# boyuanf/tensorflow_train_distributed

Hardware: AMD Instinct MI355X
Metric: images/sec (whole node) ResNet-50 bf16 MirroredStrategy at 1/2/4/8 MI355X (higher is better)
Workload: dtype bf16; 1 GPU; model=ResNet-50 v1.5, global_batch=1024, per_gpu_batch=1024, image_size=224, parallelism=dp1, optimizer=momentum-SGD 0.9, wd 5e-5, fp32 master, precision=bf16, hipgraph=True

## Files before the change

tensorflow_train_distributed_amd/csrc/kernels/conv3_halo.hip:

```cpp
#include "stream_epi.h"

namespace ttdk {
namespace {
namespace c3 {

constexpr int THR = 512;
constexpr int NW = THR / 64;

struct Pro {
  const bf16_t* x;
  const bf16_t* x2;
  const uint8_t* mask;
  const float* s;
  const float* b;
  bf16_t* side;
  uint8_t* side_mask;
};

__device__ __forceinline__ void load8f(const float* p, float (&d)[8]) {
  const f32x4_t a = *reinterpret_cast<const f32x4_t*>(p), c = *reinterpret_cast<const f32x4_t*>(p + 4);
#pragma unroll
  for (int j = 0; j < 4; ++j) {
    d[j] = a[j];
    d[4 + j] = c[j];
  }
}

template <int CP>
__device__ __forceinline__ int slot_chunk(int q) { return (q >> 3) % CP; }
template <int CP>
__device__ __forceinline__ int slot_pix(int q) { return (q & 7) + 8 * (q / (8 * CP)); }

template <int C, int BN, int TH, int W, int PRO, bool FLIP, int WM>
__global__ __launch_bounds__(THR, 1) void conv3_kernel(Pro pa, const bf16_t* __restrict__ w, EpiParams E, int H,
                                                      int N, int tiles, int nslices) {
  constexpr int BM = TH * W;
  constexpr int HR = TH + 2, HC = W + 2;
  constexpr int CP = C / 8;
  constexpr int KT = 9 * C;
  constexpr int WN = NW / WM;
  constexpr int WR = BM / WM, WC = BN / WN;
  constexpr int TM = WR / 16, TN = WC / 16;
  constexpr int NPIX = HR * HC;
  constexpr int NCH = ((NPIX + 7) / 8) * 8 * CP;
  constexpr int NA = (NCH + THR - 1) / THR;
  constexpr int SB = BN * KT * 2;
  constexpr int REG = ((NPIX * 16 + 255) / 256) * 256;
  constexpr int SH = CP * REG;
  constexpr int PITCH = BN * 2 + 16;
  constexpr int SE = BM * PITCH + NW * 3 * BN * 4;
  constexpr int SAE = SH > SE ? SH : SE;
  static_assert(C % 64 == 0 && BN % 32 == 0 && WR % 16 == 0 && WC % 16 == 0, "tile shape");
  static_assert(THR % (8 * CP) == 0, "fixed channel chunk per thread");
  static_assert(SB + SAE <= 160 * 1024, "LDS budget");
  __shared__ __attribute__((aligned(16))) char smem[SB + SAE];
  char* const sB = smem;
  char* const sA = smem + SB;

  const int b = blockIdx.x;
  const int G = gridDim.x / nslices;
  const int xcd = b & 7, rq = b >> 3;
  const int slice = rq % nslices;
  const int per_xcd = G / 8;
  const int g = xcd * per_xcd + rq / nslices;
  const int n0 = slice * BN;
  const int tid = threadIdx.x, lane = tid & 63, wave = tid >> 6;
  const int wm = wave / WN, wn = wave % WN;
  const int tiles_per_img = H / TH;

  for (int q = tid; q < BN * (KT / 8); q += THR) {
    const int row = q / (KT / 8), kk = q % (KT / 8);
    const int tap = kk / CP, cc = kk % CP;
    const int n = n0 + row;
    const int src_tap = FLIP ? 8 - tap : tap;
    const uint4 v = n < N ? ldg16(w + (static_cast<long long>(n) * 9 + src_tap) * C + cc * 8) : make_uint4(0, 0, 0, 0);
    *reinterpret_cast<uint4*>(sB + (kk >> 3) * (BN * 128) + kmaj_off(row, kk & 7)) = v;
  }

  const int ac = slot_chunk<CP>(tid);
  const bool write_side = slice == 0 && pa.side != nullptr;

  const char* abase[TM];
#pragma unroll
  for (int a = 0; a < TM; ++a) {
    const int i = wm * WR + a * 16 + (lane & 15);
    abase[a] = sA + (lane >> 4) * REG + ((i / W) * HC + (i % W)) * 16;
  }

  uint4 ra[NA], rx[PRO == 2 ? NA : 1];
  uint32_t rm[(NA + 3) / 4];
  auto load_tile = [&](int t) {
    const int img = t / tiles_per_img, h0 = (t % tiles_per_img) * TH;
#pragma unroll
    for (int i = 0; i < (NA + 3) / 4; ++i) rm[i] = 0;
#pragma unroll
    for (int i = 0; i < NA; ++i) {
      const int pix = slot_pix<CP>(tid + THR * i);
      const int hr = pix / HC, hc = pix % HC;
      const int h = h0 - 1 + hr, x = hc - 1;
      const bool ok = pix < NPIX && h >= 0 && h < H && x >= 0 && x < W;
      const long long off = ((static_cast<long long>(img) * H + h) * W + x) * C + ac * 8;
      ra[i] = ok ? ldg16(pa.x + off) : make_uint4(0, 0, 0, 0);
      if constexpr (PRO == 2) {
        rx[i] = ok ? ldg16(pa.x2 + off) : make_uint4(0, 0, 0, 0);
        rm[i >> 2] |= static_cast<uint32_t>((ok && pa.mask) ? pa.mask[off >> 3] : 0xffu) << (8 * (i & 3));
      }
    }
  };
  auto stage_tile = [&](int t) {
    const int img = t / tiles_per_img, h0 = (t % tiles_per_img) * TH;
    float k0[8], k1[8], k2[8];
    if constexpr (PRO == 1) {
      load8f(pa.s + ac * 8, k0);
      load8f(pa.b + ac * 8, k1);
    } else if constexpr (PRO == 2) {
      load8f(pa.s + ac * 8, k0);
      load8f(pa.s + C + ac * 8, k1);
      load8f(pa.s + 2 * C + ac * 8, k2);
    }
#pragma unroll
    for (int i = 0; i < NA; ++i) {
      const int pix = slot_pix<CP>(tid + THR * i);
      if (tid + THR * i >= NCH) break;
      const int hr = pix / HC, hc = pix % HC;
      const int h = h0 - 1 + hr, x = hc - 1;
      const bool ok = h >= 0 && h < H && x >= 0 && x < W;
      const bool interior = ok && hr >= 1 && hr <= TH;
      const long long off = ((static_cast<long long>(img) * H + h) * W + x) * C + ac * 8;
      uint4 v = ra[i];
      if constexpr (PRO == 1) {
        float f[8];
        unpack8(ra[i], f);
#pragma unroll
        for (int j = 0; j < 8; ++j) f[j] = relu(f[j] * k0[j] + k1[j]);
        v = ok ? pack8(f) : make_uint4(0, 0, 0, 0);
        if (write_side && interior) {
          *reinterpret_cast<uint4*>(pa.side + off) = v;
          if (pa.side_mask) {
            const uint32_t wv[4] = {v.x, v.y, v.z, v.w};
            uint32_t mb = 0;
#pragma unroll
            for (int j = 0; j < 8; ++j) {
              const uint32_t hb = (wv[j >> 1] >> (16 * (j & 1))) & 0xffffu;
              mb |= ((hb & 0x7fffu) != 0 && !(hb & 0x8000u) ? 1u : 0u) << j;
            }
            pa.side_mask[off >> 3] = static_cast<uint8_t>(mb);
          }
        }
      } else if constexpr (PRO == 2) {
        float gq[8], yf[8];
        unpack8(ra[i], gq);
        const uint32_t mb = rm[i >> 2] >> (8 * (i & 3));
#pragma unroll
        for (int j = 0; j < 8; ++j) gq[j] = (mb >> j) & 1u ? gq[j] : 0.f;
        unpack8(rx[i], yf);
#pragma unroll
        for (int j = 0; j < 8; ++j) gq[j] = k0[j] * gq[j] + k1[j] * yf[j] + k2[j];
        v = ok ? pack8(gq) : make_uint4(0, 0, 0, 0);
        if (write_side && interior) *reinterpret_cast<uint4*>(pa.side + off) = v;
      }
      *reinterpret_cast<uint4*>(sA + ac * REG + pix * 16) = v;
    }
  };

  int t = g;
  if (t < tiles) load_tile(t);
  for (; t < tiles; t += G) {
    stage_tile(t);
    __syncthreads();
    if (t + G < tiles) load_tile(t + G);
    f32x4_t acc[TM][TN];
#pragma unroll
    for (int a = 0; a < TM; ++a)
#pragma unroll
      for (int c = 0; c < TN; ++c) acc[a][c] = f32x4_t{0.f, 0.f, 0.f, 0.f};
#pragma unroll
    for (int tap = 0; tap < 9; ++tap) {
      const int tq = (tap / 3) * HC + (tap % 3);
#pragma unroll
      for (int kc = 0; kc < C / 32; ++kc) {
        const int kglob = tap * C + kc * 32;
        const char* pB = sB + (kglob >> 6) * (BN * 128);
        const int kchunk = ((kglob & 63) >> 3) + (lane >> 4);
        bf16x8_t af[TM], bfr[TN];
#pragma unroll
        for (int c = 0; c < TN; ++c) bfr[c] = lds_read_b128(pB + kmaj_off(wn * WC + c * 16 + (lane & 15), kchunk));
#pragma unroll
        for (int a = 0; a < TM; ++a) af[a] = lds_read_b128(abase[a] + kc * 4 * REG + tq * 16);
#pragma unroll
        for (int a = 0; a < TM; ++a)
#pragma unroll
          for (int c = 0; c < TN; ++c) acc[a][c] = __builtin_amdgcn_mfma_f32_16x16x32_bf16(bfr[c], af[a], acc[a][c], 0, 0, 0);
      }
    }
    __syncthreads();
    sepi::stage_acc<TM, TN, WR, WC, PITCH>(sA, acc, wm, wn, lane, epi_alpha(E));
    __syncthreads();
    constexpr int ECPR = BN / 8;
    constexpr int RPP = THR / ECPR;
    const int m0 = t * BM;
    const int c = tid % ECPR, r0 = tid / ECPR;
    const int n = n0 + c * 8;
    const bool nfull = n + 8 <= N;
    const bool vst = nfull && (E.ldo & 7) == 0;
    float bias8[8], s8[8], q8[8], r8[8];
#pragma unroll
    for (int j = 0; j < 8; ++j) {
      bias8[j] = (E.bias && n + j < N) ? E.bias[n + j] : 0.f;
      s8[j] = q8[j] = r8[j] = 0.f;
    }
    const int M = tiles * BM;
    if (E.beta || E.residual || E.by)
      epi_rows<BM, RPP, PITCH, true, 2>(E, sA, c, r0, n, m0, M, N, vst, vst, bias8, s8, q8, r8);
    else
      epi_rows<BM, RPP, PITCH, false>(E, sA, c, r0, n, m0, M, N, vst, vst, bias8, s8, q8, r8);
    if (E.stat)
      sepi::tile_stats<BN, NW, THR, ECPR>(E, reinterpret_cast<float*>(sA + BM * PITCH), s8, q8, r8, c, lane, wave, tid,
                                          n0, N, t);
    else
      __syncthreads();
  }
}

template <int C, int BN, int TH, int W, int PRO, bool FLIP, int WM>
hipError_t launch(const Pro& pa, const bf16_t* w, const EpiParams& E, int Nimg, int H, int N, hipStream_t st) {
  const int nsl = N / BN;
  const int tiles = Nimg * (H / TH);
  int per_xcd = big::device_cus() / (8 * nsl);
  if (per_xcd < 1) per_xcd = 1;
  const int need = ceil_div(tiles, 8);
  if (per_xcd > need) per_xcd = need;
  hipLaunchKernelGGL((conv3_kernel<C, BN, TH, W, PRO, FLIP, WM>), dim3(8 * nsl * per_xcd), dim3(THR), 0, st, pa, w, E, H, N,
                     tiles, nsl);
  return hipGetLastError();
}

inline int pick_th(int C, int N, int W, int pro) {
  if (C == 64 && N == 64 && W == 56) return pro == 2 ? 4 : 8;
  return 0;
}

template <int PRO, bool FLIP>
hipError_t dispatch(const Pro& pa, const bf16_t* w, const EpiParams& E, int Nimg, int H, int W, int C, int N,
                    hipStream_t st) {
  if (C == 64 && N == 64 && W == 56) {
    if constexpr (PRO == 2) return launch<64, 64, 4, 56, PRO, FLIP, 2>(pa, w, E, Nimg, H, N, st);
    else return launch<64, 64, 8, 56, PRO, FLIP, 4>(pa, w, E, Nimg, H, N, st);
  }
  return hipErrorInvalidValue;
}

}

namespace c3s {

constexpr int THR = 512;
constexpr int NW = THR / 64;

__device__ __forceinline__ void dma16(const void* src, uint32_t lds_) {
  const uint32_t lds = __builtin_amdgcn_readfirstlane(lds_);
  unsigned keep;
  asm volatile("s_mov_b32 %0, m0\n\ts_mov_b32 m0, %2\n\ts_nop 0\n\tglobal_load_lds_dwordx4 %1, off\n\ts_mov_b32 m0, %0"
               : "=&s"(keep) : "v"(src), "s"(lds) : "memory");
}
__device__ __forceinline__ uint32_t lds_addr(const char* p) {
  typedef __attribute__((address_space(3))) const char lds_char_t;
  return (uint32_t)(size_t)(lds_char_t*)(p);
}

template <int N>
__device__ __forceinline__ void wait_vm() {
  asm volatile("s_waitcnt vmcnt(%0)" ::"n"(N) : "memory");
}

template <int C, int BN, int TR, int H, int W, int PRO, bool FLIP>
__global__ __launch_bounds__(THR, 1) void conv3s_kernel(c3::Pro pa, const bf16_t* __restrict__ w, EpiParams E,
                                                       int rows_total, int N, int tiles) {
  constexpr int WM = 2, WN = NW / WM;
  constexpr int BM = TR * W;
  constexpr int WR = BM / WM, WC = BN / WN;
  constexpr int TM = WR / 16, TN = WC / 16;
  constexpr int HS = TR + 4;
  constexpr int HC = W + 2;
  constexpr int NPIX = HS * HC;
  constexpr int CP = C / 8;
  constexpr int NCH = ((NPIX + 7) / 8) * 8 * CP;
  constexpr int NA = (NCH + THR - 1) / THR;
  constexpr int REG = ((NPIX * 16 + 255) / 256) * 256;
  constexpr int SH = CP * REG;
  constexpr int SBT = BN * C * 2;
  constexpr int PITCH = BN * 2 + 16;
  constexpr int SE = BM * PITCH + NW * 3 * BN * 4;
  constexpr int SAE = SH > SE ? SH : SE;
  constexpr int NDMA = SBT / 16 / THR;
  static_assert(PRO != 2 && C % 64 == 0 && BN % (16 * WN) == 0 && WR % 16 == 0 && TR <= H, "tile shape");
  static_assert(THR % (8 * CP) == 0 && SBT % (16 * THR) == 0, "staging / DMA mapping");
  static_assert(SAE + 2 * SBT <= 160 * 1024, "LDS budget");
  __shared__ __attribute__((aligned(16))) char smem[SAE + 2 * SBT];
  char* const sA = smem;
  char* const sBb = smem + SAE;

  const int b = blockIdx.x;
  const int G = gridDim.x;
  const int g = (b & 7) * (G / 8) + (b >> 3);
  const int tid = threadIdx.x, lane = tid & 63, wave = tid >> 6;
  const int wm = wave / WN, wn = wave % WN;
  const int ac = c3::slot_chunk<CP>(tid);
  const bool write_side = pa.side != nullptr;
  const int nimg = rows_total / H;

  auto dma_tap = [&](int tap, int buf) {
    const int stap = FLIP ? 8 - tap : tap;
    char* dst = sBb + buf * SBT;
#pragma unroll
    for (int i = 0; i < NDMA; ++i) {
      const int L = (i * NW + wave) * 64 + lane;
      const int sub = L / (BN * 8), p = L % (BN * 8), row = p >> 3, j = p & 7;
      const int sc = j ^ ((row >> 1) & 7);
      dma16(w + (static_cast<long long>(row) * 9 + stap) * C + (sub * 8 + sc) * 8,
            lds_addr(dst + (i * NW + wave) * 1024));
    }
  };
  struct Geo {
    int i0, h0, n0, n1;
  };
  auto geo = [&](int t) {
    Geo q;
    const int R0 = t * TR, R1 = min(R0 + TR, rows_total);
    q.i0 = R0 / H;
    q.h0 = R0 - q.i0 * H;
    q.n0 = min(R1, (q.i0 + 1) * H) - R0;
    q.n1 = R1 - R0 - q.n0;
    return q;
  };
  auto slot_src = [&](const Geo& q, int s, int& img, int& h, bool& interior) {
    if (s < q.n0 + 2) {
      img = q.i0;
      h = q.h0 - 1 + s;
      interior = s >= 1 && s <= q.n0;
      return true;
    }
    const int u = s - (q.n0 + 2);
    img = q.i0 + 1;
    h = u - 1;
    interior = u >= 1 && u <= q.n1;
    return q.n1 > 0 && u < q.n1 + 2;
  };

  uint4 ra[NA];
  auto load_tile = [&](int t) {
    const Geo q = geo(t);
#pragma unroll
    for (int i = 0; i < NA; ++i) {
      const int qq = tid + THR * i;
      const int pix = c3::slot_pix<CP>(qq);
      const int s = pix / HC, x = pix % HC - 1;
      int img, h;
      bool interior;
      const bool ok = qq < NCH && slot_src(q, s, img, h, interior) && h >= 0 && h < H && x >= 0 && x < W;
      const long long off = ((static_cast<long long>(img) * H + h) * W + x) * C + ac * 8;
      ra[i] = ldg16(ok ? pa.x + off : reinterpret_cast<const bf16_t*>(big::g_zero));
    }
  };
  auto stage_tile = [&](int t) {
    const Geo q = geo(t);
    float k0[8], k1[8];
    if constexpr (PRO == 1) {
      c3::load8f(pa.s + ac * 8, k0);
      c3::load8f(pa.b + ac * 8, k1);
    }
#pragma unroll
    for (int i = 0; i < NA; ++i) {
      const int qq = tid + THR * i;
      if (qq >= NCH) break;
      const int pix = c3::slot_pix<CP>(qq);
      const int s = pix / HC, x = pix % HC - 1;
      int img, h;
      bool interior;
      const bool ok = slot_src(q, s, img, h, interior) && h >= 0 && h < H && x >= 0 && x < W;
      uint4 v = ok ? ra[i] : make_uint4(0, 0, 0, 0);
      if constexpr (PRO == 1) {
        const long long off = ((static_cast<long long>(img) * H + h) * W + x) * C + ac * 8;
        float f[8];
        unpack8(ra[i], f);
#pragma unroll
        for (int j = 0; j < 8; ++j) f[j] = relu(f[j] * k0[j] + k1[j]);
        v = ok ? pack8(f) : make_uint4(0, 0, 0, 0);
        if (write_side && ok && interior) {
          *reinterpret_cast<uint4*>(pa.side + off) = v;
          if (pa.side_mask) {
            const uint32_t wv[4] = {v.x, v.y, v.z, v.w};
            uint32_t mb = 0;
#pragma unroll
            for (int j = 0; j < 8; ++j) {
              const uint32_t hb = (wv[j >> 1] >> (16 * (j & 1))) & 0xffffu;
              mb |= ((hb & 0x7fffu) != 0 && !(hb & 0x8000u) ? 1u : 0u) << j;
            }
            pa.side_mask[off >> 3] = static_cast<uint8_t>(mb);
          }
        }
      }
      *reinterpret_cast<uint4*>(sA + ac * REG + pix * 16) = v;
    }
  };

  int bcur = 0;
  int t = g;
  if (t < tiles) {
    dma_tap(0, 0);
    load_tile(t);
  }
  for (; t < tiles; t += G) {
    const Geo q = geo(t);
    int abase[TM];
#pragma unroll
    for (int a = 0; a < TM; ++a) {
      const int i = wm * WR + a * 16 + (lane & 15);
      const int j = i / W, col = i % W;
      abase[a] = (lane >> 4) * REG + ((j + (j >= q.n0 ? 2 : 0)) * HC + col) * 16;
    }
    stage_tile(t);
    wait_vm<0>();
    __syncthreads();
    const bool more = t + G < tiles;
    f32x4_t acc[TM][TN];
#pragma unroll
    for (int a = 0; a < TM; ++a)
#pragma unroll
      for (int c = 0; c < TN; ++c) acc[a][c] = f32x4_t{0.f, 0.f, 0.f, 0.f};
#pragma unroll 1
    for (int tap = 0; tap < 9; ++tap) {
      const int bnext = bcur ^ 1;
      if (tap < 8) dma_tap(tap + 1, bnext);
      else if (more) dma_tap(0, bnext);
      const char* sBc = sBb + bcur * SBT;
      const int tq = ((tap / 3) * HC + (tap % 3)) * 16;
#pragma unroll
      for (int kc = 0; kc < C / 32; ++kc) {
        const int kglob = kc * 32;
        const char* pB = sBc + (kglob >> 6) * (BN * 128);
        const int kchunk = ((kglob & 63) >> 3) + (lane >> 4);
        bf16x8_t af[TM], bfr[TN];
#pragma unroll
        for (int c = 0; c < TN; ++c) bfr[c] = lds_read_b128(pB + kmaj_off(wn * WC + c * 16 + (lane & 15), kchunk));
#pragma unroll
        for (int a = 0; a < TM; ++a) af[a] = lds_read_b128(sA + abase[a] + kc * 4 * REG + tq);
#pragma unroll
        for (int a = 0; a < TM; ++a)
#pragma unroll
          for (int c = 0; c < TN; ++c) acc[a][c] = __builtin_amdgcn_mfma_f32_16x16x32_bf16(bfr[c], af[a], acc[a][c], 0, 0, 0);
      }
      wait_vm<0>();
      __syncthreads();
      bcur = bnext;
    }
    sepi::stage_acc<TM, TN, WR, WC, PITCH>(sA, acc, wm, wn, lane, epi_alpha(E));
    if (more) load_tile(t + G);
    __syncthreads();
    constexpr int ECPR = BN / 8;
    constexpr int RPP = THR / ECPR;
    const int m0 = t * BM;
    const int c = tid % ECPR, r0 = tid / ECPR;
    const int n = c * 8;
    const bool vst = (E.ldo & 7) == 0;
    float bias8[8], s8[8], q8[8], r8[8];
#pragma unroll
    for (int j = 0; j < 8; ++j) {
      bias8[j] = E.bias ? E.bias[n + j] : 0.f;
      s8[j] = q8[j] = r8[j] = 0.f;
    }
    const int M = rows_total * W;
    if (E.beta || E.residual || E.by)
      epi_rows<BM, RPP, PITCH, true, 2>(E, sA, c, r0, n, m0, M, N, vst, vst, bias8, s8, q8, r8);
    else
      epi_rows<BM, RPP, PITCH, false>(E, sA, c, r0, n, m0, M, N, vst, vst, bias8, s8, q8, r8);
    if (E.stat)
      sepi::tile_stats<BN, NW, THR, ECPR>(E, reinterpret_cast<float*>(sA + BM * PITCH), s8, q8, r8, c, lane, wave, tid,
                                          0, N, t);
    else
      __syncthreads();
    (void)nimg;
  }
}

template <int PRO, bool FLIP>
hipError_t launch(const c3::Pro& pa, const bf16_t* w, const EpiParams& E, int Nimg, int N, hipStream_t st) {
  const int rows = Nimg * 28;
  const int tiles = ceil_div(rows, 8);
  int G = big::device_cus() / 8 * 8;
  if (G < 8) G = 8;
  const int need = ceil_div(tiles, 8) * 8;
  if (G > need) G = need;
  hipLaunchKernelGGL((conv3s_kernel<128, 128, 8, 28, 28, PRO, FLIP>), dim3(G), dim3(THR), 0, st, pa, w, E, rows, N,
                     tiles);
  return hipGetLastError();
}

inline bool fits(int H, int W, int C, int N, int pro) { return C == 128 && N == 128 && H == 28 && W == 28 && pro != 2; }

}
}
}

using namespace ttdk;

namespace {
int& conv3_s3_flag() {
  static int on = getenv_int("TTD_CONV3_S3", 1);
  return on;
}
}

TTDK_EXPORT int ttdk_set_conv3_s3(int on) {
  const int old = conv3_s3_flag();
  conv3_s3_flag() = on;
  return old;
}

TTDK_EXPORT int ttdk_conv3_rows(int H, int W, int C, int N, int pro) {
  if (conv3_s3_flag() && c3s::fits(H, W, C, N, pro)) return 8 * W;
  const int th = c3::pick_th(C, N, W, pro);
  return (th && H % th == 0) ? th * W : 0;
}

TTDK_EXPORT int ttdk_conv3_halo(const bf16_t* x, const bf16_t* x2, const uint8_t* mask_in, const float* s,
                                const float* b, bf16_t* side, uint8_t* side_mask, int pro, int flip, const bf16_t* w,
                                int Nimg, int H, int W, int C, int N, const TtdkEpilogue* epi, hipStream_t st) {
  if (ttdk_conv3_rows(H, W, C, N, pro) == 8 * W && c3s::fits(H, W, C, N, pro)) {
    if ((reinterpret_cast<uintptr_t>(x) & 15) || (reinterpret_cast<uintptr_t>(w) & 15)) return hipErrorInvalidValue;
    const EpiParams e = to_epi(epi);
    if (e.mode != 0 || e.remap || e.bH || e.ldo != N || e.residual || e.by2) return hipErrorInvalidValue;
    if (pro == 1 && (!s || !b)) return hipErrorInvalidValue;
    if (side_mask && pro != 1) return hipErrorInvalidValue;
    const c3::Pro pa{x, nullptr, nullptr, s, b, side, side_mask};
    if (pro == 0 && !flip) return c3s::launch<0, false>(pa, w, e, Nimg, N, st);
    if (pro == 0 && flip) return c3s::launch<0, true>(pa, w, e, Nimg, N, st);
    if (pro == 1 && !flip) return c3s::launch<1, false>(pa, w, e, Nimg, N, st);
    return hipErrorInvalidValue;
  }
  const int th = c3::pick_th(C, N, W, pro);
  if (!th || H % th || (reinterpret_cast<uintptr_t>(x) & 15) || pro < 0 || pro > 2) return hipErrorInvalidValue;
  const EpiParams e = to_epi(epi);
  if (e.mode != 0 || e.remap || e.bH || e.ldo != N || e.residual || e.by2) return hipErrorInvalidValue;
  if (pro == 1 && (!s || !b)) return hipErrorInvalidValue;
  if (pro == 2 && (!s || !x2)) return hipErrorInvalidValue;
  if (side_mask && pro != 1) return hipErrorInvalidValue;
  const c3::Pro pa{x, x2, mask_in, s, b, side, side_mask};
#define C3_CASE(P_, F_) \
  if (pro == P_ && (flip != 0) == F_) return c3::dispatch<P_, F_>(pa, w, e, Nimg, H, W, C, N, st);
  C3_CASE(0, false)
  C3_CASE(1, false)
  C3_CASE(0, true)
  C3_CASE(2, true)
#undef C3_CASE
  return hipErrorInvalidValue;
}
```

tensorflow_train_distributed_amd/ops/gemm.py:

```python
from __future__ import annotations

import ctypes

import torch

from . import _lib, _plan

ACT_NONE, ACT_RELU, ACT_GELU, ACT_TANH, ACT_DGELU = 0, 1, 2, 3, 4

import os as _os
_LOG = [] if _os.environ.get("TTD_GEMM_LOG") else None


def gemm_log(reset=False):
    out = list(_LOG or [])
    if reset and _LOG is not None:
        _LOG.clear()
    return out


def _log(kind, M, N, K, splits=1):
    if _LOG is not None:
        _LOG.append((kind, int(M), int(N), int(K), int(splits)))
    _lib.label((kind, int(M), int(N), int(K)))
# ... 67 lines not shown
        raise ValueError("gemm out must be [%d, %d] row-major (got %s strides %s)" % (M, N, tuple(out.shape),
                                                                                   out.stride()))
    _log("gemm_%s%s" % ("t" if trans_a else "n", "t" if trans_b else "n"), M, N, K, splits)
    a_kmajor = 0 if trans_a else 1
    lda = a.stride(0)
    b_kmajor = 1 if trans_b else 0
    ldb = b.stride(0)
    if out.dtype == torch.float32:
        splits = effective_splits(K, splits)
        if splits > 1:
            if not out.is_contiguous():
                raise ValueError("split-K output must be contiguous")
            ws = torch.empty((splits, M, N), dtype=torch.float32, device=a.device)
            _lib.call("ttdk_gemm_bf16_splitk", a.data_ptr(), lda, a_kmajor, b.data_ptr(), ldb, b_kmajor, M, N, K,
                      splits, ws.data_ptr(), out.data_ptr(), beta, float(alpha), int(tile[0]), int(tile[1]),
                      _lib.stream())
            return out
        e = _epi(out, mode=2, beta=beta, alpha=alpha)
    else:
        e = _epi(out, bias=bias, residual=residual, act=act, beta=beta, alpha=alpha, aux=aux, stat=stat)
    _lib.call("ttdk_gemm_bf16", a.data_ptr(), lda, a_kmajor, b.data_ptr(), ldb, b_kmajor, M, N, K, 1,
              tile[0], tile[1], ctypes.byref(e), _lib.stream())
    return out


_lib.register({"ttdk_gemm4w_bf16": [_lib.P, _lib.L, _lib.P, _lib.L, _lib.I, _lib.I, _lib.I, _lib.E, _lib.P],
               "ttdk_set_g4_sched": [_lib.I], "ttdk_set_g4_group": [_lib.I],
               "ttdk_set_g4_stagger": [_lib.I]})


def set_g4_stagger(v: int) -> int:
    return int(_lib.query("ttdk_set_g4_stagger", int(v)))


def set_g4_group(v: int) -> int:
    return int(_lib.query("ttdk_set_g4_group", int(v)))


def set_g4_sched(v: int) -> int:
    return int(_lib.query("ttdk_set_g4_sched", int(v)))


def gemm4w(a, b, *, out=None, bias=None, act=ACT_NONE, residual=None, beta=0, alpha=1.0, aux=None):
    _check2d(a, torch.bfloat16, "a")
    _check2d(b, torch.bfloat16, "b")
    M, K = a.shape
    N, Kb = b.shape
    if K != Kb:
        raise ValueError("gemm4w inner dims differ: %d vs %d" % (K, Kb))
    if out is None:
        out = torch.empty((M, N), dtype=torch.bfloat16, device=a.device)
    e = _epi(out, bias=bias, residual=residual, act=act, beta=beta, alpha=alpha, aux=aux)
    _log("gemm4w", M, N, K, 1)
    _lib.call("ttdk_gemm4w_bf16", a.data_ptr(), a.stride(0), b.data_ptr(), b.stride(0), M, N, K, ctypes.byref(e),
              _lib.stream())
    return out


_lib.register({"ttdk_gemm_bf16_batched": [_lib.P, _lib.L, _lib.L, _lib.I, _lib.P, _lib.L, _lib.L, _lib.I, _lib.P,
                                          _lib.L, _lib.L, _lib.I, _lib.I, _lib.I, _lib.I, _lib.I, _lib.P],
               "ttdk_gemm_f32_batched": [_lib.P, _lib.L, _lib.L, _lib.I, _lib.P, _lib.L, _lib.L, _lib.I, _lib.P,
                                         _lib.L, _lib.L, _lib.I, _lib.I, _lib.I, _lib.I, _lib.P]})


def gemm_batched(a, b, *, trans_a=False, trans_b=False, out_dtype=torch.float32):
    if a.dim() != 3 or b.dim() != 3 or a.shape[0] != b.shape[0]:
        raise ValueError("gemm_batched needs [B, ., .] operands with equal batch, got %s and %s"
                         % (tuple(a.shape), tuple(b.shape)))
    a = a.contiguous()
    b = b.contiguous()
    Bt = a.shape[0]
    M, K = (a.shape[2], a.shape[1]) if trans_a else (a.shape[1], a.shape[2])
    Kb, N = (b.shape[2], b.shape[1]) if trans_b else (b.shape[1], b.shape[2])
    if K != Kb:
        raise ValueError("gemm_batched inner dims differ: %d vs %d" % (K, Kb))
    _log("gemm_batched", M, N, K, Bt)
    if a.dtype == torch.float32 and b.dtype == torch.float32:
        out = torch.empty((Bt, M, N), dtype=torch.float32, device=a.device)
        _lib.call("ttdk_gemm_f32_batched", a.data_ptr(), a.stride(1), a.stride(0), int(trans_a), b.data_ptr(),
                  b.stride(1), b.stride(0), int(trans_b), out.data_ptr(), N, M * N, M, N, K, Bt, _lib.stream())
        return out
    _check(a, torch.bfloat16, "a")
    _check(b, torch.bfloat16, "b")
    out = torch.empty((Bt, M, N), dtype=out_dtype, device=a.device)
    _lib.call("ttdk_gemm_bf16_batched", a.data_ptr(), a.stride(1), a.stride(0), 0 if trans_a else 1, b.data_ptr(),
              b.stride(1), b.stride(0), 1 if trans_b else 0, out.data_ptr(), N, M * N,
              1 if out_dtype == torch.float32 else 0, M, N, K, Bt, _lib.stream())
    return out


def wgrad_bias_ok(M, N, K, splits) -> bool:
    if M % 8 or N % 8 or K % 64:
        return False
    if int(_lib.query("ttdk_gemm_wgrad_bias_ws", int(M), int(N), int(K), int(splits))) < 0:
        return False
    kt = K // 64
    return -(-kt // _plan.clamp_splits(kt, int(splits))) >= 16


def gemm_wgrad_bias(dy, x, out, bias_out, splits=1, beta=0, alpha=1.0):
    _check2d(dy, torch.bfloat16, "dy")
    _check2d(x, torch.bfloat16, "x")
    K, M = dy.shape
    K2, N = x.shape
    if K != K2:
        raise ValueError("gemm_wgrad_bias: token dims differ (%d vs %d)" % (K, K2))
    if tuple(out.shape) != (M, N) or out.dtype != torch.float32 or not out.is_contiguous():
        raise ValueError("gemm_wgrad_bias: out must be a contiguous fp32 [%d, %d]" % (M, N))
    if bias_out.numel() != M or bias_out.dtype != torch.float32 or not bias_out.is_contiguous():
        raise ValueError("gemm_wgrad_bias: bias_out must be a contiguous fp32 [%d]" % M)
    nws = int(_lib.query("ttdk_gemm_wgrad_bias_ws", M, N, K, int(splits)))
    if nws < 0:
        raise ValueError("gemm_wgrad_bias: shape %dx%dx%d not on the 256-wide kernel" % (M, N, K))
    ws = torch.empty(nws, dtype=torch.float32, device=dy.device)
    _log("wgrad_bias", M, N, K, splits)
    _lib.call("ttdk_gemm_wgrad_bias", dy.data_ptr(), dy.stride(0), x.data_ptr(), x.stride(0), M, N, K, int(splits),
              ws.data_ptr(), out.data_ptr(), int(beta), float(alpha), bias_out.data_ptr(), _lib.stream())
    return out, bias_out


def gemm4t(dy, x, out=None, bias_out=None, *, splits=1, beta=0, alpha=1.0):
    _check2d(dy, torch.bfloat16, "dy")
    _check2d(x, torch.bfloat16, "x")
    K, M = dy.shape
    K2, N = x.shape
    if K != K2:
        raise ValueError("gemm4t: token dims differ (%d vs %d)" % (K, K2))
    if out is None:
        out = torch.empty((M, N), dtype=torch.float32, device=dy.device)
    if tuple(out.shape) != (M, N) or out.dtype != torch.float32 or not out.is_contiguous():
        raise ValueError("gemm4t: out must be a contiguous fp32 [%d, %d]" % (M, N))
    if bias_out is not None and (bias_out.numel() != M or bias_out.dtype != torch.float32
                                 or not bias_out.is_contiguous()):
        raise ValueError("gemm4t: bias_out must be a contiguous fp32 [%d]" % M)
    nws = int(_lib.query("ttdk_gemm4t_ws", M, N, K, int(splits)))
    if nws < 0:
        raise ValueError("gemm4t does not take M=%d N=%d K=%d (K a multiple of 64 >= 128, M / N multiples "
                         "of 8, operands < 2 GiB, TTD_G4T on)" % (M, N, K))
    ws = torch.empty(max(nws, 1), dtype=torch.float32, device=dy.device)
    _log("gemm4t", M, N, K, splits)
    _lib.call("ttdk_gemm4t_wgrad", dy.data_ptr(), dy.stride(0), x.data_ptr(), x.stride(0), M, N, K, int(splits),
              ws.data_ptr(), out.data_ptr(), int(beta), float(alpha), _lib.ptr(bias_out), _lib.stream())
    return out


_C3 = _os.environ.get("TTD_CONV3", "1") != "0"


_lib.register({"ttdk_set_conv3_s3": [_lib.I]})


def set_conv3_s3(on: bool) -> bool:
    return bool(_lib.query("ttdk_set_conv3_s3", 1 if on else 0))


def conv3_rows(H, W, C, N, pro=0):
    return int(_lib.query("ttdk_conv3_rows", int(H), int(W), int(C), int(N), int(pro))) if _C3 else 0


def conv3_halo(x, w, *, prologue=None, flip=False, out=None, stat=False, bn_stat=None):
    _check(x, torch.bfloat16, "x")
    _check(w, torch.bfloat16, "w")
    Nimg, H, W, C = x.shape
    Co = w.shape[0]
    if tuple(w.shape) != (Co, 3, 3, C):
        raise ValueError("conv3_halo: filter must be [%d, 3, 3, %d], got %s" % (Co, C, tuple(w.shape)))
    pro_code = 0 if prologue is None else {"bn_fwd": 1, "bn_bwd": 2}.get(prologue[0], -1)
    bm = conv3_rows(H, W, C, Co, max(pro_code, 0))
    if not bm:
        raise ValueError("conv3_halo: shape %s -> %d not compiled in" % (tuple(x.shape), Co))
    if out is None:
        out = torch.empty((Nimg, H, W, Co), dtype=torch.bfloat16, device=x.device)
    T = -(-Nimg * H * W // bm)
    partial = None
    by = bmask = None
    if stat or bn_stat is not None:
        partial = torch.empty((T, 2, Co), dtype=torch.float32, device=x.device)
    if bn_stat is not None:
        by, bmask = bn_stat
        _check(by, torch.bfloat16, "bn_stat y")
    e = _epi(out, ldo=Co, stat=partial, by=by, bmask=bmask)
    P = _lib.ptr
    pro, x2, mask_in, s, b, side, side_mask = 0, None, None, None, None, None, None
    if prologue is not None:
        if prologue[0] == "bn_fwd":
            _, s, b, side, side_mask = prologue
            pro = 1
        elif prologue[0] == "bn_bwd":
            _, x2, mask_in, s, side = prologue
            pro = 2
        else:
            raise ValueError("unknown prologue %r" % (prologue[0],))
    _log("c3_%s" % ("dgrad" if flip else "fwd"), Nimg * H * W, Co, 9 * C)
    _lib.call("ttdk_conv3_halo", x.data_ptr(), P(x2), P(mask_in), P(s), P(b), P(side), P(side_mask), pro, int(flip),
              w.data_ptr(), Nimg, H, W, C, Co, ctypes.byref(e), _lib.stream())
    if partial is not None:
        return out, partial, T
    return out


def gemm_f32(a, b, *, trans_a=False, trans_b=False, out=None, bias=None, beta=0):
    _check2d(a, torch.float32, "a")
    _check2d(b, torch.float32, "b")
    M, K = (a.shape[1], a.shape[0]) if trans_a else a.shape
    Kb, N = (b.shape[1], b.shape[0]) if trans_b else b.shape
    if K != Kb:
        raise ValueError("gemm inner dims differ: %d vs %d" % (K, Kb))
    if out is None:
        if beta:
            raise ValueError("beta=1 needs an out tensor")
        out = torch.empty((M, N), dtype=torch.float32, device=a.device)
    elif out.dtype != torch.float32 or tuple(out.shape) != (M, N) or out.stride(-1) != 1:
        raise ValueError("gemm_f32 out must be fp32 [%d, %d] row-major" % (M, N))
    if bias is not None:
        _check(bias, torch.float32, "bias")
    _log("gemm_f32_%s%s" % ("t" if trans_a else "n", "t" if trans_b else "n"), M, N, K, 1)
    _lib.call("ttdk_gemm_f32", a.data_ptr(), a.stride(0), int(trans_a), b.data_ptr(), b.stride(0), int(trans_b),
              out.data_ptr(), out.stride(0), _lib.ptr(bias), int(bool(beta)), M, N, K, _lib.stream())
    return out


BIG_WGRAD_WGS = int(_os.environ.get("TTD_WGRAD_WGS", "128"))


def gemm_wgrad_splits(M, N, K, target_blocks=1024, min_ktiles=8, big_wgs=None):
    bbn = big_bn(M, N, K)
    if bbn:
        tiles = -(-M // 256) * -(-N // bbn)
        return max(1, min((K // 64) // 32, -(-(big_wgs or BIG_WGRAD_WGS) // tiles)))
    bm, bn = _plan.pick_tile(M, N)
    tiles = -(-M // bm) * -(-N // bn)
    ktiles = -(-K // 64)
    return max(1, min(ktiles // min_ktiles, -(-target_blocks // tiles)))


def conv_geom(x_shape, w_shape, stride, padding, dilation=(1, 1)):
    N, H, W, C = x_shape
    K, R, S, Cw = w_shape
    if C != Cw:
        raise ValueError("channel mismatch %d vs %d" % (C, Cw))
    sh, sw = stride
    ph, pw = padding
    dh, dw = dilation
    P = (H + 2 * ph - dh * (R - 1) - 1) // sh + 1
    Q = (W + 2 * pw - dw * (S - 1) - 1) // sw + 1
    g = _lib.ConvGeom(N, H, W, C, K, R, S, P, Q, sh, sw, ph, pw, dh, dw)
    return g


def pw_rows(N, K, dma=False):
    return int(_lib.query("ttdk_pw_rows", int(N), int(K), int(bool(dma))))


_PW = _os.environ.get("TTD_PW", "1") != "0"


def pw_ok(M, N, K):
    return _PW and pw_rows(N, K) > 0 and N * K <= 65536


def pw_wgrad_fusable(M, N, K, dma=True):
    return _PW and int(_lib.query("ttdk_pw_wgrad_slabs", int(M), int(N), int(K), int(bool(dma)), 0)) > 0


def pw_conv(x, w, *, prologue=None, out=None, stat=False, beta=0, residual=None, bn_stat=None, bn_stat2=None,
            beta_s2=None, wgrad=None, max_wgs=0, fold_stream=None, keep=None):
    _check(x, torch.bfloat16, "x")
    _check(w, torch.bfloat16, "w")
    K = x.shape[-1]
    M = x.numel() // K
    N = w.shape[0]
    if w.numel() != N * K:
        raise ValueError("pw_conv: weight must be [N, K] = [%d, %d] (got %s)" % (N, K, tuple(w.shape)))
    dma = bool(beta or bn_stat is not None) and residual is None and bn_stat2 is None
    bm = pw_rows(N, K, dma)
    if not bm:
        raise ValueError("pw_conv: N=%d K=%d not handled by the streaming kernel" % (N, K))
    if out is None:
        out = torch.empty(tuple(x.shape[:-1]) + (N,), dtype=torch.bfloat16, device=x.device)
    T = -(-M // bm)
    partial = partial2 = None
    by = bmask = by2 = None
    if stat or bn_stat is not None:
        partial = torch.empty((T, 2, N), dtype=torch.float32, device=x.device)
    if bn_stat is not None:
        by, bmask = bn_stat
        _check(by, torch.bfloat16, "bn_stat y")
        if bn_stat2 is not None:
            by2 = bn_stat2
            partial2 = torch.empty((T, 2, N), dtype=torch.float32, device=x.device)
    e = _epi(out, ldo=N, beta=beta, residual=residual, stat=partial, by=by, bmask=bmask, by2=by2, stat2=partial2,
             beta_s2=beta_s2 if beta else None)
    P = _lib.ptr
    pro, x2, mask_in, s, b, rs, rb, side, side_mask = 0, None, None, None, None, None, None, None, None
    if prologue is not None:
        if prologue[0] == "bn_fwd":
            _, s, b, x2, rs, rb, side, side_mask = prologue
            pro = 1
        elif prologue[0] == "bn_bwd":
            _, x2, mask_in, s, side = prologue
            pro = 2
        else:
            raise ValueError("pw_conv: unknown prologue %r" % (prologue[0],))
    _log("pw_%s" % ("fwd" if pro != 2 else "dgrad"), M, N, K)
    if wgrad is not None:
        xw, dw = wgrad[0], wgrad[1]
# ... 571 lines not shown
```

Baseline: 15620 images/sec.

## Interleave next-tile halo loads across conv3 taps and pin fragment scheduling

Adds a SCHED template variant (on by default via TTD_CONV3_SCHED) to the 3x3 halo conv kernels. In the stride kernel it spreads the next tile's halo global loads across the nine tap iterations, issuing two slots per tap, with partial vmcnt waits in place of a bulk load after the MMA loop. It also precomputes per-lane weight DMA source pointers. Both kernels insert sched_barrier fences around LDS fragment reads and MFMA groups, and use an opaque tid to stop the compiler hoisting address math. The aim is to hide global load latency behind the tap loop and keep register pressure steady. The risks are extra register use from full unrolling and weaker compiler scheduling.

```diff
diff --git a/tensorflow_train_distributed_amd/csrc/kernels/conv3_halo.hip b/tensorflow_train_distributed_amd/csrc/kernels/conv3_halo.hip
--- a/tensorflow_train_distributed_amd/csrc/kernels/conv3_halo.hip
+++ b/tensorflow_train_distributed_amd/csrc/kernels/conv3_halo.hip
@@ -31,7 +31,21 @@
 template <int CP>
 __device__ __forceinline__ int slot_pix(int q) { return (q & 7) + 8 * (q / (8 * CP)); }
 
-template <int C, int BN, int TH, int W, int PRO, bool FLIP, int WM>
+template <int SCHED>
+__device__ __forceinline__ int fresh(int tid) {
+  if constexpr (SCHED != 0) {
+    asm volatile("" : "+v"(tid));
+    __builtin_assume(tid >= 0 && tid < THR);
+  }
+  return tid;
+}
+
+template <int SCHED>
+__device__ __forceinline__ void frag_fence() {
+  if constexpr (SCHED != 0) __builtin_amdgcn_sched_barrier(0);
+}
+
+template <int C, int BN, int TH, int W, int PRO, bool FLIP, int WM, int SCHED>
 __global__ __launch_bounds__(THR, 1) void conv3_kernel(Pro pa, const bf16_t* __restrict__ w, EpiParams E, int H,
                                                       int N, int tiles, int nslices) {
   constexpr int BM = TH * W;
@@ -91,11 +105,12 @@
   uint32_t rm[(NA + 3) / 4];
   auto load_tile = [&](int t) {
     const int img = t / tiles_per_img, h0 = (t % tiles_per_img) * TH;
+    const int ft = fresh<SCHED>(tid);
 #pragma unroll
     for (int i = 0; i < (NA + 3) / 4; ++i) rm[i] = 0;
 #pragma unroll
     for (int i = 0; i < NA; ++i) {
-      const int pix = slot_pix<CP>(tid + THR * i);
+      const int pix = slot_pix<CP>(ft + THR * i);
       const int hr = pix / HC, hc = pix % HC;
       const int h = h0 - 1 + hr, x = hc - 1;
       const bool ok = pix < NPIX && h >= 0 && h < H && x >= 0 && x < W;
@@ -118,10 +133,11 @@
       load8f(pa.s + C + ac * 8, k1);
       load8f(pa.s + 2 * C + ac * 8, k2);
     }
+    const int ft = fresh<SCHED>(tid);
 #pragma unroll
     for (int i = 0; i < NA; ++i) {
-      const int pix = slot_pix<CP>(tid + THR * i);
-      if (tid + THR * i >= NCH) break;
+      const int pix = slot_pix<CP>(ft + THR * i);
+      if (ft + THR * i >= NCH) break;
       const int hr = pix / HC, hc = pix % HC;
       const int h = h0 - 1 + hr, x = hc - 1;
       const bool ok = h >= 0 && h < H && x >= 0 && x < W;
@@ -184,13 +200,20 @@
         const int kchunk = ((kglob & 63) >> 3) + (lane >> 4);
         bf16x8_t af[TM], bfr[TN];
 #pragma unroll
-        for (int c = 0; c < TN; ++c) bfr[c] = lds_read_b128(pB + kmaj_off(wn * WC + c * 16 + (lane & 15), kchunk));
-#pragma unroll
-        for (int a = 0; a < TM; ++a) af[a] = lds_read_b128(abase[a] + kc * 4 * REG + tq * 16);
+        for (int c = 0; c < TN; ++c) {
+          bfr[c] = lds_read_b128(pB + kmaj_off(wn * WC + c * 16 + (lane & 15), kchunk));
+          frag_fence<SCHED>();
+        }
+#pragma unroll
+        for (int a = 0; a < TM; ++a) {
+          af[a] = lds_read_b128(abase[a] + kc * 4 * REG + tq * 16);
+          frag_fence<SCHED>();
+        }
 #pragma unroll
         for (int a = 0; a < TM; ++a)
 #pragma unroll
           for (int c = 0; c < TN; ++c) acc[a][c] = __builtin_amdgcn_mfma_f32_16x16x32_bf16(bfr[c], af[a], acc[a][c], 0, 0, 0);
+        frag_fence<SCHED>();
       }
     }
     __syncthreads();
@@ -222,7 +245,7 @@
   }
 }
 
-template <int C, int BN, int TH, int W, int PRO, bool FLIP, int WM>
+template <int C, int BN, int TH, int W, int PRO, bool FLIP, int WM, int SCHED>
 hipError_t launch(const Pro& pa, const bf16_t* w, const EpiParams& E, int Nimg, int H, int N, hipStream_t st) {
   const int nsl = N / BN;
   const int tiles = Nimg * (H / TH);
@@ -230,8 +253,8 @@
   if (per_xcd < 1) per_xcd = 1;
   const int need = ceil_div(tiles, 8);
   if (per_xcd > need) per_xcd = need;
-  hipLaunchKernelGGL((conv3_kernel<C, BN, TH, W, PRO, FLIP, WM>), dim3(8 * nsl * per_xcd), dim3(THR), 0, st, pa, w, E, H, N,
-                     tiles, nsl);
+  hipLaunchKernelGGL((conv3_kernel<C, BN, TH, W, PRO, FLIP, WM, SCHED>), dim3(8 * nsl * per_xcd), dim3(THR), 0, st, pa, w,
+                     E, H, N, tiles, nsl);
   return hipGetLastError();
 }
 
@@ -240,12 +263,12 @@
   return 0;
 }
 
-template <int PRO, bool FLIP>
+template <int PRO, bool FLIP, int SCHED>
 hipError_t dispatch(const Pro& pa, const bf16_t* w, const EpiParams& E, int Nimg, int H, int W, int C, int N,
                     hipStream_t st) {
   if (C == 64 && N == 64 && W == 56) {
-    if constexpr (PRO == 2) return launch<64, 64, 4, 56, PRO, FLIP, 2>(pa, w, E, Nimg, H, N, st);
-    else return launch<64, 64, 8, 56, PRO, FLIP, 4>(pa, w, E, Nimg, H, N, st);
+    if constexpr (PRO == 2) return launch<64, 64, 4, 56, PRO, FLIP, 2, SCHED>(pa, w, E, Nimg, H, N, st);
+    else return launch<64, 64, 8, 56, PRO, FLIP, 4, SCHED>(pa, w, E, Nimg, H, N, st);
   }
   return hipErrorInvalidValue;
 }
@@ -272,8 +295,16 @@
 __device__ __forceinline__ void wait_vm() {
   asm volatile("s_waitcnt vmcnt(%0)" ::"n"(N) : "memory");
 }
-
-template <int C, int BN, int TR, int H, int W, int PRO, bool FLIP>
+__device__ __forceinline__ void wait_vm_upto(int n) {
+  switch (n) {
+    case 1: wait_vm<1>(); break;
+    case 2: wait_vm<2>(); break;
+    case 3: wait_vm<3>(); break;
+    default: wait_vm<0>(); break;
+  }
+}
+
+template <int C, int BN, int TR, int H, int W, int PRO, bool FLIP, int SCHED>
 __global__ __launch_bounds__(THR, 1) void conv3s_kernel(c3::Pro pa, const bf16_t* __restrict__ w, EpiParams E,
                                                        int rows_total, int N, int tiles) {
   constexpr int WM = 2, WN = NW / WM;
@@ -309,16 +340,30 @@
   const bool write_side = pa.side != nullptr;
   const int nimg = rows_total / H;
 
+  const bf16_t* wsrc[NDMA];
+#pragma unroll
+  for (int i = 0; i < NDMA; ++i) {
+    const int L = (i * NW + wave) * 64 + lane;
+    const int sub = L / (BN * 8), p = L % (BN * 8), row = p >> 3, j = p & 7;
+    const int sc = j ^ ((row >> 1) & 7);
+    wsrc[i] = w + static_cast<long long>(row) * 9 * C + (sub * 8 + sc) * 8;
+  }
   auto dma_tap = [&](int tap, int buf) {
     const int stap = FLIP ? 8 - tap : tap;
     char* dst = sBb + buf * SBT;
 #pragma unroll
     for (int i = 0; i < NDMA; ++i) {
-      const int L = (i * NW + wave) * 64 + lane;
-      const int sub = L / (BN * 8), p = L % (BN * 8), row = p >> 3, j = p & 7;
-      const int sc = j ^ ((row >> 1) & 7);
-      dma16(w + (static_cast<long long>(row) * 9 + stap) * C + (sub * 8 + sc) * 8,
-            lds_addr(dst + (i * NW + wave) * 1024));
+      if constexpr (SCHED != 0) {
+        int off = stap * C;
+        asm volatile("" : "+s"(off));
+        dma16(wsrc[i] + off, lds_addr(dst + (i * NW + wave) * 1024));
+      } else {
+        const int L = (i * NW + wave) * 64 + lane;
+        const int sub = L / (BN * 8), p = L % (BN * 8), row = p >> 3, j = p & 7;
+        const int sc = j ^ ((row >> 1) & 7);
+        dma16(w + (static_cast<long long>(row) * 9 + stap) * C + (sub * 8 + sc) * 8,
+              lds_addr(dst + (i * NW + wave) * 1024));
+      }
     }
   };
   struct Geo {
@@ -348,19 +393,21 @@
   };
 
   uint4 ra[NA];
+  auto load_slot = [&](const Geo& q, int ft, int i) {
+    const int qq = ft + THR * i;
+    const int pix = c3::slot_pix<CP>(qq);
+    const int s = pix / HC, x = pix % HC - 1;
+    int img, h;
+    bool interior;
+    const bool ok = qq < NCH && slot_src(q, s, img, h, interior) && h >= 0 && h < H && x >= 0 && x < W;
+    const long long off = ((static_cast<long long>(img) * H + h) * W + x) * C + ac * 8;
+    ra[i] = ldg16(ok ? pa.x + off : reinterpret_cast<const bf16_t*>(big::g_zero));
+  };
   auto load_tile = [&](int t) {
     const Geo q = geo(t);
-#pragma unroll
-    for (int i = 0; i < NA; ++i) {
-      const int qq = tid + THR * i;
-      const int pix = c3::slot_pix<CP>(qq);
-      const int s = pix / HC, x = pix % HC - 1;
-      int img, h;
-      bool interior;
-      const bool ok = qq < NCH && slot_src(q, s, img, h, interior) && h >= 0 && h < H && x >= 0 && x < W;
-      const long long off = ((static_cast<long long>(img) * H + h) * W + x) * C + ac * 8;
-      ra[i] = ldg16(ok ? pa.x + off : reinterpret_cast<const bf16_t*>(big::g_zero));
-    }
+    const int ft = c3::fresh<SCHED>(tid);
+#pragma unroll
+    for (int i = 0; i < NA; ++i) load_slot(q, ft, i);
   };
   auto stage_tile = [&](int t) {
     const Geo q = geo(t);
@@ -369,9 +416,10 @@
       c3::load8f(pa.s + ac * 8, k0);
       c3::load8f(pa.b + ac * 8, k1);
     }
+    const int ft = c3::fresh<SCHED>(tid);
 #pragma unroll
     for (int i = 0; i < NA; ++i) {
-      const int qq = tid + THR * i;
+      const int qq = ft + THR * i;
       if (qq >= NCH) break;
       const int pix = c3::slot_pix<CP>(qq);
       const int s = pix / HC, x = pix % HC - 1;
@@ -409,6 +457,7 @@
   if (t < tiles) {
     dma_tap(0, 0);
     load_tile(t);
+    if constexpr (SCHED != 0) wait_vm<0>();
   }
   for (; t < tiles; t += G) {
     const Geo q = geo(t);
@@ -420,7 +469,7 @@
       abase[a] = (lane >> 4) * REG + ((j + (j >= q.n0 ? 2 : 0)) * HC + col) * 16;
     }
     stage_tile(t);
-    wait_vm<0>();
+    if constexpr (SCHED == 0) wait_vm<0>();
     __syncthreads();
     const bool more = t + G < tiles;
     f32x4_t acc[TM][TN];
@@ -428,11 +477,22 @@
     for (int a = 0; a < TM; ++a)
 #pragma unroll
       for (int c = 0; c < TN; ++c) acc[a][c] = f32x4_t{0.f, 0.f, 0.f, 0.f};
-#pragma unroll 1
+    constexpr int HPT = 2;
+    static_assert(HPT * 8 >= NA, "the halo loads are all retired by the wait of the last tap");
+    const Geo qn = geo(SCHED != 0 && more ? t + G : t);
+#pragma unroll(SCHED != 0 ? 9 : 1)
     for (int tap = 0; tap < 9; ++tap) {
       const int bnext = bcur ^ 1;
       if (tap < 8) dma_tap(tap + 1, bnext);
       else if (more) dma_tap(0, bnext);
+      const int h0 = tap * HPT < NA ? tap * HPT : NA, h1 = h0 + HPT < NA ? h0 + HPT : NA;
+      if constexpr (SCHED != 0) {
+        if (more) {
+          const int ft = c3::fresh<SCHED>(tid);
+#pragma unroll
+          for (int i = h0; i < h1; ++i) load_slot(qn, ft, i);
+        }
+      }
       const char* sBc = sBb + bcur * SBT;
       const int tq = ((tap / 3) * HC + (tap % 3)) * 16;
 #pragma unroll
@@ -442,20 +502,29 @@
         const int kchunk = ((kglob & 63) >> 3) + (lane >> 4);
         bf16x8_t af[TM], bfr[TN];
 #pragma unroll
-        for (int c = 0; c < TN; ++c) bfr[c] = lds_read_b128(pB + kmaj_off(wn * WC + c * 16 + (lane & 15), kchunk));
-#pragma unroll
-        for (int a = 0; a < TM; ++a) af[a] = lds_read_b128(sA + abase[a] + kc * 4 * REG + tq);
+        for (int c = 0; c < TN; ++c) {
+          bfr[c] = lds_read_b128(pB + kmaj_off(wn * WC + c * 16 + (lane & 15), kchunk));
+          c3::frag_fence<SCHED>();
+        }
+#pragma unroll
+        for (int a = 0; a < TM; ++a) {
+          af[a] = lds_read_b128(sA + abase[a] + kc * 4 * REG + tq);
+          c3::frag_fence<SCHED>();
+        }
 #pragma unroll
         for (int a = 0; a < TM; ++a)
 #pragma unroll
           for (int c = 0; c < TN; ++c) acc[a][c] = __builtin_amdgcn_mfma_f32_16x16x32_bf16(bfr[c], af[a], acc[a][c], 0, 0, 0);
+        c3::frag_fence<SCHED>();
       }
-      wait_vm<0>();
+      if constexpr (SCHED != 0) wait_vm_upto(more ? h1 - h0 : 0);
+      else wait_vm<0>();
       __syncthreads();
       bcur = bnext;
     }
     sepi::stage_acc<TM, TN, WR, WC, PITCH>(sA, acc, wm, wn, lane, epi_alpha(E));
-    if (more) load_tile(t + G);
+    if constexpr (SCHED == 0)
+      if (more) load_tile(t + G);
     __syncthreads();
     constexpr int ECPR = BN / 8;
     constexpr int RPP = THR / ECPR;
@@ -483,7 +552,7 @@
   }
 }
 
-template <int PRO, bool FLIP>
+template <int PRO, bool FLIP, int SCHED>
 hipError_t launch(const c3::Pro& pa, const bf16_t* w, const EpiParams& E, int Nimg, int N, hipStream_t st) {
   const int rows = Nimg * 28;
   const int tiles = ceil_div(rows, 8);
@@ -491,8 +560,8 @@
   if (G < 8) G = 8;
   const int need = ceil_div(tiles, 8) * 8;
   if (G > need) G = need;
-  hipLaunchKernelGGL((conv3s_kernel<128, 128, 8, 28, 28, PRO, FLIP>), dim3(G), dim3(THR), 0, st, pa, w, E, rows, N,
-                     tiles);
+  hipLaunchKernelGGL((conv3s_kernel<128, 128, 8, 28, 28, PRO, FLIP, SCHED>), dim3(G), dim3(THR), 0, st, pa, w, E, rows,
+                     N, tiles);
   return hipGetLastError();
 }
 
@@ -509,6 +578,16 @@
   static int on = getenv_int("TTD_CONV3_S3", 1);
   return on;
 }
+int& conv3_sched_flag() {
+  static int on = getenv_int("TTD_CONV3_SCHED", 1);
+  return on;
+}
+}
+
+TTDK_EXPORT int ttdk_set_conv3_sched(int on) {
+  const int old = conv3_sched_flag();
+  conv3_sched_flag() = on ? 1 : 0;
+  return old;
 }
 
 TTDK_EXPORT int ttdk_set_conv3_s3(int on) {
@@ -526,6 +605,7 @@
 TTDK_EXPORT int ttdk_conv3_halo(const bf16_t* x, const bf16_t* x2, const uint8_t* mask_in, const float* s,
                                 const float* b, bf16_t* side, uint8_t* side_mask, int pro, int flip, const bf16_t* w,
                                 int Nimg, int H, int W, int C, int N, const TtdkEpilogue* epi, hipStream_t st) {
+  const int sched = conv3_sched_flag();
   if (ttdk_conv3_rows(H, W, C, N, pro) == 8 * W && c3s::fits(H, W, C, N, pro)) {
     if ((reinterpret_cast<uintptr_t>(x) & 15) || (reinterpret_cast<uintptr_t>(w) & 15)) return hipErrorInvalidValue;
     const EpiParams e = to_epi(epi);
@@ -533,9 +613,13 @@
     if (pro == 1 && (!s || !b)) return hipErrorInvalidValue;
     if (side_mask && pro != 1) return hipErrorInvalidValue;
     const c3::Pro pa{x, nullptr, nullptr, s, b, side, side_mask};
-    if (pro == 0 && !flip) return c3s::launch<0, false>(pa, w, e, Nimg, N, st);
-    if (pro == 0 && flip) return c3s::launch<0, true>(pa, w, e, Nimg, N, st);
-    if (pro == 1 && !flip) return c3s::launch<1, false>(pa, w, e, Nimg, N, st);
+#define C3S_CASE(P_, F_)              \
+  if (pro == P_ && (flip != 0) == F_) \
+    return sched ? c3s::launch<P_, F_, 1>(pa, w, e, Nimg, N, st) : c3s::launch<P_, F_, 0>(pa, w, e, Nimg, N, st);
+    C3S_CASE(0, false)
+    C3S_CASE(0, true)
+    C3S_CASE(1, false)
+#undef C3S_CASE
     return hipErrorInvalidValue;
   }
   const int th = c3::pick_th(C, N, W, pro);
@@ -546,8 +630,10 @@
   if (pro == 2 && (!s || !x2)) return hipErrorInvalidValue;
   if (side_mask && pro != 1) return hipErrorInvalidValue;
   const c3::Pro pa{x, x2, mask_in, s, b, side, side_mask};
-#define C3_CASE(P_, F_) \
-  if (pro == P_ && (flip != 0) == F_) return c3::dispatch<P_, F_>(pa, w, e, Nimg, H, W, C, N, st);
+#define C3_CASE(P_, F_)                                                           \
+  if (pro == P_ && (flip != 0) == F_)                                             \
+    return sched ? c3::dispatch<P_, F_, 1>(pa, w, e, Nimg, H, W, C, N, st)        \
+                 : c3::dispatch<P_, F_, 0>(pa, w, e, Nimg, H, W, C, N, st);
   C3_CASE(0, false)
   C3_CASE(1, false)
   C3_CASE(0, true)
diff --git a/tensorflow_train_distributed_amd/ops/gemm.py b/tensorflow_train_distributed_amd/ops/gemm.py
--- a/tensorflow_train_distributed_amd/ops/gemm.py
+++ b/tensorflow_train_distributed_amd/ops/gemm.py
@@ -243,6 +243,13 @@
 
 def set_conv3_s3(on: bool) -> bool:
     return bool(_lib.query("ttdk_set_conv3_s3", 1 if on else 0))
+
+
+_lib.register({"ttdk_set_conv3_sched": [_lib.I]})
+
+
+def set_conv3_sched(new: bool) -> bool:
+    return bool(_lib.query("ttdk_set_conv3_sched", 1 if new else 0))
 
 
 def conv3_rows(H, W, C, N, pro=0):
```

Result: faster. 15880 images/sec (median of 6 runs) (+1.7%).
